# dspcraft/dsc

Hardware: AMD Instinct MI355X
Metric: batched 1-D rfft GSamples/s (higher is better)
Workload: dtype f32

## Files before the change

### dsc_amd/csrc/fft_c2c_32k.hip

```cpp
#define DSC_R2C64K_HELPERS_ONLY 1
#include "fft_r2c_64k.hip"

namespace {

template<bool INV, bool CAST>
__global__ __launch_bounds__(1024) void c2c32k_kernel(const f2 *__restrict__ z, f2 *__restrict__ Z, int batch, const f2 *__restrict__ aux,
                                                      int in_pitch, int in_len) {
    constexpr int EB = CAST ? 4 : 8;
    auto sample = [](__amdgpu_buffer_rsrc_t r, int voff, int soff) {
        if constexpr (CAST) return cf{__builtin_bit_cast(float, __builtin_amdgcn_raw_buffer_load_b32(r, voff, soff, kStream)), 0.0f};
        else return load_c(r, voff, soff);
    };
    extern __shared__ __attribute__((aligned(16))) float lds[];
    float *plane = lds;
    f2 *T = (f2 *) (lds + kPlaneFloats);
    fill_twiddle_table(T, aux);
    const int wave_sgpr = __builtin_amdgcn_readfirstlane(threadIdx.x >> 6);
    constexpr float kScale = 1.0f / (float) kM;

    cf v[32];
    {
        const int row0 = blockIdx.x;
        const __amdgpu_buffer_rsrc_t r0 = __builtin_amdgcn_make_buffer_rsrc(
            (void *) ((const char *) z + (size_t) row0 * in_pitch * EB), 0, row0 < batch ? in_len * EB : 0, 0x00020000);
        const int load_off = thread_id(wave_sgpr) * EB;
#pragma unroll
        for (int a = 0; a < 32; ++a) v[a] = sample(r0, load_off, a * 1024 * EB);
    }
    for (int row = blockIdx.x; row < batch; row += gridDim.x) {
        const int next_row = row + gridDim.x;
        const __amdgpu_buffer_rsrc_t rnext = __builtin_amdgcn_make_buffer_rsrc(
            (void *) ((const char *) z + (size_t) next_row * in_pitch * EB), 0, next_row < batch ? in_len * EB : 0, 0x00020000);
        const __amdgpu_buffer_rsrc_t rout = __builtin_amdgcn_make_buffer_rsrc((void *) (Z + (size_t) row * kM), 0, kM * 8, 0x00020000);
        three_passes<INV>(v, plane, T, aux, wave_sgpr, wave_sgpr, false, false);
        if (INV) {
#pragma unroll
            for (int p = 0; p < 32; ++p) v[p] = cf{v[p].x * kScale, v[p].y * kScale};
        }
        const int load_off = thread_id(wave_sgpr) * EB;
        staged_time_store(v, plane, rout, wave_sgpr, [&](bool first_half) {
            if (first_half) {
#pragma unroll
                for (int a = 0; a < 16; ++a) v[2 * a] = sample(rnext, load_off, a * 1024 * EB);
            } else {
#pragma unroll
                for (int a = 16; a < 32; ++a) v[2 * (a - 16) + 1] = sample(rnext, load_off, a * 1024 * EB);
            }
        });
        unzip_rows(v);
    }
}

}

void dsc_launch_fft32k_c32(const void *z, void *Z, int batch, int in_pitch, int in_len, bool inverse, bool cast, const void *aux, int n_cu,
                           hipStream_t stream) {
    if (batch <= 0) return;
    static unsigned long long attr_devices = 0;
    if (dsc_first_use_on_device(attr_devices)) {
        DSC_KERNEL_CHECK(hipFuncSetAttribute((const void *) c2c32k_kernel<false, false>, hipFuncAttributeMaxDynamicSharedMemorySize, kLdsBytes));
        DSC_KERNEL_CHECK(hipFuncSetAttribute((const void *) c2c32k_kernel<true, false>, hipFuncAttributeMaxDynamicSharedMemorySize, kLdsBytes));
        DSC_KERNEL_CHECK(hipFuncSetAttribute((const void *) c2c32k_kernel<false, true>, hipFuncAttributeMaxDynamicSharedMemorySize, kLdsBytes));
        DSC_KERNEL_CHECK(hipFuncSetAttribute((const void *) c2c32k_kernel<true, true>, hipFuncAttributeMaxDynamicSharedMemorySize, kLdsBytes));
    }
    const int grid = batch < n_cu ? batch : n_cu;
#define C2C32K(INV, CAST) DSC_LAUNCH((c2c32k_kernel<INV, CAST>), dim3(grid), dim3(1024), kLdsBytes, stream, (const f2 *) z, (f2 *) Z, batch, (const f2 *) aux, in_pitch, in_len)
    if (inverse) { if (cast) C2C32K(true, true); else C2C32K(true, false); }
    else         { if (cast) C2C32K(false, true); else C2C32K(false, false); }
#undef C2C32K
}
```

### dsc_amd/csrc/fft_r2c_64k.hip

```cpp
#include "kernels.h"

#include <hip/hip_runtime.h>

#include <cmath>
#include <cstdlib>
#include <utility>

namespace {

typedef float f2 __attribute__((ext_vector_type(2)));

struct cf { float x, y; };
__device__ __forceinline__ cf operator+(cf a, cf b) { return cf{a.x + b.x, a.y + b.y}; }
__device__ __forceinline__ cf operator-(cf a, cf b) { return cf{a.x - b.x, a.y - b.y}; }
__device__ __forceinline__ cf to_cf(f2 a) { return cf{a.x, a.y}; }
__device__ __forceinline__ f2 to_f2(cf a) { return f2{a.x, a.y}; }

constexpr int kM = 32768;
constexpr int kPlaneFloats = 1024 * 34;
constexpr int kLdsBytes = kPlaneFloats * 4 + 1024 * 8;
constexpr int kTabEntries = 1024;

constexpr int kAuxW1024 = 0, kAuxW32768 = 1024, kAuxW65536 = 2048, kAuxEntries = 3072;

// ... 144 lines not shown
__device__ __forceinline__ void dit_stage(cf (&v)[32], std::integer_sequence<int, G...>) {
    (dit_group<INV, S, G>(v, std::make_integer_sequence<int, (32 >> S)>{}), ...);
}

template<bool INV>
__device__ __forceinline__ void dft32(cf (&v)[32]) {
    dit_stage<INV, 1>(v, std::make_integer_sequence<int, 1>{});
    dit_stage<INV, 2>(v, std::make_integer_sequence<int, 2>{});
    dit_stage<INV, 3>(v, std::make_integer_sequence<int, 4>{});
    dit_stage<INV, 4>(v, std::make_integer_sequence<int, 8>{});
    dit_stage<INV, 5>(v, std::make_integer_sequence<int, 16>{});
}

template<bool INV>
__device__ __forceinline__ void dft32_head(cf (&v)[32]) {
    dit_stage<INV, 1>(v, std::make_integer_sequence<int, 1>{});
    dit_stage<INV, 2>(v, std::make_integer_sequence<int, 2>{});
}
template<bool INV, int Q>
__device__ __forceinline__ void dft32_quarter(cf (&v)[32]) {
    dit_stage<INV, 3>(v, std::integer_sequence<int, Q>{});
    dit_stage<INV, 4>(v, std::integer_sequence<int, 2 * Q, 2 * Q + 1>{});
    dit_stage<INV, 5>(v, std::integer_sequence<int, 4 * Q, 4 * Q + 1, 4 * Q + 2, 4 * Q + 3>{});
}
#endif

typedef unsigned int u2 __attribute__((ext_vector_type(2)));
typedef unsigned int u4 __attribute__((ext_vector_type(4)));
typedef float f4 __attribute__((ext_vector_type(4)));

#ifndef DSC_LDS_SPLIT_READS
#define DSC_LDS_SPLIT_READS 1
#endif
__device__ __forceinline__ f2 lds_read_b64(const f2 *p) {
#if DSC_LDS_SPLIT_READS
    return *(const volatile __attribute__((address_space(3))) f2 *) p;
#else
    return *p;
#endif
}

__device__ __forceinline__ void lds_barrier() {
    __builtin_amdgcn_fence(__ATOMIC_RELEASE, "workgroup", "local");
    __builtin_amdgcn_s_barrier();
    __builtin_amdgcn_fence(__ATOMIC_ACQUIRE, "workgroup", "local");
}

__device__ __forceinline__ float bperm(int byte_addr, float x) {
    return __int_as_float(__builtin_amdgcn_ds_bpermute(byte_addr, __float_as_int(x)));
}

__device__ __forceinline__ int column_of(int wave, int lane) {
    int kp = lane < 32 ? 32 * wave + lane : 1024 - 32 * wave - (63 - lane);
    return kp == 1024 ? 512 : kp;
}

#ifdef DSC_R2C64K_PROBE
#define PROBE_ARGS , int io_on
#define PROBE_NULL , 1
#define IO_ON io_on
#else
#define PROBE_ARGS
#define PROBE_NULL
#define IO_ON 1
#endif

__device__ __forceinline__ int thread_id(int wave_sgpr) {
    int zero;
    asm volatile("v_mov_b32 %0, 0" : "=v"(zero));
    const int lane = __builtin_amdgcn_mbcnt_hi(-1, __builtin_amdgcn_mbcnt_lo(-1, zero));
    return (wave_sgpr << 6) | lane;
}

#ifndef DSC_STREAM_AUX
#define DSC_STREAM_AUX 2
#endif
constexpr int kStream = DSC_STREAM_AUX;
__device__ __forceinline__ cf load_c(__amdgpu_buffer_rsrc_t r, int voff, int soff) {
    return to_cf(__builtin_bit_cast(f2, __builtin_amdgcn_raw_buffer_load_b64(r, voff, soff, kStream)));
}
#ifndef DSC_FILTER_EARLY_LOADS
#define DSC_FILTER_EARLY_LOADS 4
#endif
#ifndef DSC_IRFFT_PIN_PASS3
#define DSC_IRFFT_PIN_PASS3 1
#endif
#ifndef DSC_IRFFT_EARLY_PAIRS
#define DSC_IRFFT_EARLY_PAIRS 4
#endif
#ifndef DSC_IRFFT_LOAD_AUX
#define DSC_IRFFT_LOAD_AUX 0
#endif
__device__ __forceinline__ cf load_c_spec(__amdgpu_buffer_rsrc_t r, int voff, int soff) {
    return to_cf(__builtin_bit_cast(f2, __builtin_amdgcn_raw_buffer_load_b64(r, voff, soff, DSC_IRFFT_LOAD_AUX)));
}
__device__ __forceinline__ cf load_c_cached(__amdgpu_buffer_rsrc_t r, int voff, int soff) {
    return to_cf(__builtin_bit_cast(f2, __builtin_amdgcn_raw_buffer_load_b64(r, voff, soff, 0)));
}
template<int POLICY>
__device__ __forceinline__ void store_c(cf a, __amdgpu_buffer_rsrc_t r, int voff, int soff) {
    __builtin_amdgcn_raw_buffer_store_b64(__builtin_bit_cast(u2, to_f2(a)), r, voff, soff, POLICY);
}

__device__ __forceinline__ void fill_twiddle_table(f2 *T, const f2 *aux) {
    const int t = threadIdx.x;
    T[t] = aux[kAuxW1024 + (t >> 5) * (t & 31)];
    __syncthreads();
}

constexpr int kCPitch = 33;
static_assert(512 * kCPitch * 8 <= kPlaneFloats * 4, "the step buffer lives inside the plane");

__host__ __device__ constexpr int class_of(int k) { return (k ^ (k >> 1)) & 1; }
__host__ __device__ constexpr int index_in_class(int k) { return ((k >> 2) << 1) | (k & 1); }
static_assert(class_of(br5(0)) == 0 && class_of(br5(7)) == 0 && class_of(br5(24)) == 0 && class_of(br5(31)) == 0 &&
              class_of(br5(8)) == 1 && class_of(br5(23)) == 1, "class 0 = quarters 0 and 3 of a dft32 output");

__device__ __forceinline__ int reader_column(int t) {
    const int a = t >> 5;
    return (t & 31) | ((((a >> 3) | ((a & 7) << 2))) << 5);
}
__device__ __forceinline__ int spectrum_wave(int wave_sgpr) { return (wave_sgpr >> 2) | ((wave_sgpr & 3) << 2); }

template<int Q>
__device__ __forceinline__ void quarter_write(f2 *buf, int wbase, const cf (&v)[32]) {
    int wbase_hi = wbase + 8 * (32 * kCPitch);
    asm("" : "+v"(wbase_hi));
    f2 *lo8 = buf + wbase;
    f2 *hi8 = buf + wbase_hi;
#pragma unroll
    for (int p = 8 * Q; p < 8 * Q + 8; ++p)
        if (index_in_class(br5(p)) < 8) lo8[index_in_class(br5(p)) * (32 * kCPitch)] = to_f2(v[p]);
#pragma unroll
    for (int p = 8 * Q; p < 8 * Q + 8; ++p)
        if (index_in_class(br5(p)) >= 8) hi8[(index_in_class(br5(p)) - 8) * (32 * kCPitch)] = to_f2(v[p]);
}

__device__ __forceinline__ void step_read(const f2 *buf, int row, cf (&dst)[32]) {
    const f2 *r = buf + __mul24(row, kCPitch);
#pragma unroll
    for (int m = 0; m < 32; ++m) dst[m] = to_cf(lds_read_b64(r + m));
}

__device__ __forceinline__ void pin(cf (&v)[32]) {
#pragma unroll
    for (int p = 0; p < 32; p += 8)
        asm volatile("" : "+v"(v[p].x), "+v"(v[p].y), "+v"(v[p + 1].x), "+v"(v[p + 1].y), "+v"(v[p + 2].x), "+v"(v[p + 2].y), "+v"(v[p + 3].x),
                     "+v"(v[p + 3].y), "+v"(v[p + 4].x), "+v"(v[p + 4].y), "+v"(v[p + 5].x), "+v"(v[p + 5].y), "+v"(v[p + 6].x), "+v"(v[p + 6].y),
                     "+v"(v[p + 7].x), "+v"(v[p + 7].y));
}

template<typename Finish>
__device__ __forceinline__ void exchange(f2 *buf, int wbase, int rclass, int rrow, cf (&src)[32], cf (&dst)[32], Finish finish) {
    pin(src);
    lds_barrier();
    finish(std::integral_constant<int, 0>{});
    quarter_write<0>(buf, wbase, src);
    finish(std::integral_constant<int, 3>{});
    quarter_write<3>(buf, wbase, src);
    lds_barrier();
    cf r[32];
    if (rclass == 0) step_read(buf, rrow, r);
    finish(std::integral_constant<int, 1>{});
    lds_barrier();
    quarter_write<1>(buf, wbase, src);
    finish(std::integral_constant<int, 2>{});
    quarter_write<2>(buf, wbase, src);
    lds_barrier();
    if (rclass != 0) step_read(buf, rrow, r);
#pragma unroll
    for (int m = 0; m < 32; ++m) dst[m] = r[m];
}

struct no_hook { __device__ __forceinline__ void operator()() const {} };

template<bool INV, typename Hook = no_hook>
__device__ __forceinline__ void three_passes(cf (&v)[32], float *plane, const f2 *T, const f2 *aux, int wave_sgpr, int col_wave,
                                             bool mirrored_in, bool mirrored_out, Hook before_pass3 = Hook{}) {
    f2 *buf = (f2 *) plane;
    const int wave_class = ((wave_sgpr >> 2) ^ (wave_sgpr >> 3)) & 1;
    dft32_head<INV>(v);
    cf u[32];
    {
        const int t = thread_id(wave_sgpr);
        const int col = mirrored_in ? column_of(col_wave, t & 63) : t;
        const int hi = col >> 5;
        const f2 *th = T + hi;
        const int rc = reader_column(t);
        exchange(buf, __mul24(col & 31, kCPitch) + hi, wave_class, (index_in_class(rc >> 5) << 5) | (rc & 31), v, u, [&](auto Q) {
            constexpr int kQ = decltype(Q)::value;
            dft32_quarter<INV, kQ>(v);
#pragma unroll
            for (int p = 8 * kQ; p < 8 * kQ + 8; ++p) {
                if (p == 0) continue;
                const cf w = to_cf(th[32 * br5(p)]);
                v[p] = INV ? cmul_conj(v[p], w) : cmul(v[p], w);
            }
        });
    }
    dft32_head<INV>(u);
    {
        const int t = thread_id(wave_sgpr);
        const int rc = reader_column(t);
        const int hi = rc >> 5, lo = rc & 31;
        const cf tw2_base = to_cf(aux[kAuxW32768 + __mul24(hi, lo)]);
        const f2 *tl = T + lo;
        const int col_out = mirrored_out ? column_of(col_wave, t & 63) : rc;
        const int k2 = col_out >> 5;
        const int rclass = mirrored_out ? class_of(k2) : wave_class;
        exchange(buf, __mul24(hi, kCPitch) + lo, rclass, (index_in_class(k2) << 5) | (col_out & 31), u, v, [&](auto Q) {
            constexpr int kQ = decltype(Q)::value;
            dft32_quarter<INV, kQ>(u);
#ifdef DSC_DFT32_DIF
            constexpr bool kSumsOnly = false;
#else
            constexpr bool kSumsOnly = true;
#endif
#pragma unroll
            for (int p = 8 * kQ; p < 8 * kQ + 8; ++p) {
                const cf w = p == 0 ? tw2_base : cmul(tw2_base, to_cf(tl[32 * br5(p)]));
                if (kSumsOnly && p < 4) u[p] = twiddle_mul_second_fused<INV>(u[p], w);
                else u[p] = INV ? cmul_conj(u[p], w) : cmul(u[p], w);
            }
        });
    }
    before_pass3();
    dft32<INV>(v);
}

__device__ __forceinline__ void real_pair(cf p, cf q, cf wq, float hs, cf &out_k, cf &out_mk) {
    const cf s = cf{p.x + q.x, p.y - q.y};
    const cf d = cf{p.x - q.x, p.y + q.y};
    const cf wd = cmul(d, wq);
    out_k = cf{hs * s.x + wd.x, hs * s.y + wd.y};
    out_mk = cf{hs * s.x - wd.x, wd.y - hs * s.y};
}

__device__ __forceinline__ int partner_byte_addr(int wave, int lane) {
    return ((wave == 0 && (lane == 63 || lane == 0)) ? lane : 63 - lane) * 4;
}

#ifndef DSC_R2C64K_HELPERS_ONLY
__global__ __launch_bounds__(1024) void rfft64k_kernel(const float *__restrict__ x, f2 *__restrict__ X, int batch,
                                                       const f2 *__restrict__ aux, int in_pitch, int in_len PROBE_ARGS) {
    extern __shared__ __attribute__((aligned(16))) float lds[];
    float *plane = lds;
    f2 *T = (f2 *) (lds + kPlaneFloats);
    fill_twiddle_table(T, aux);

    const int wave_sgpr = __builtin_amdgcn_readfirstlane(threadIdx.x >> 6);

    cf v[32];
    {
        const int row0 = blockIdx.x;
        const __amdgpu_buffer_rsrc_t r0 = __builtin_amdgcn_make_buffer_rsrc(
            (void *) (x + (size_t) row0 * in_pitch), 0, row0 < batch ? in_len * 4 * IO_ON : 0, 0x00020000);
        const int load_off = thread_id(wave_sgpr) * 8;
#pragma unroll
        for (int j1 = 0; j1 < 32; ++j1) v[j1] = load_c(r0, load_off, j1 * 8192);
    }

    for (int row = blockIdx.x; row < batch; row += gridDim.x) {
        const int next_row = row + gridDim.x;
        const __amdgpu_buffer_rsrc_t rnext = __builtin_amdgcn_make_buffer_rsrc(
            (void *) (x + (size_t) next_row * in_pitch), 0, next_row < batch ? in_len * 4 * IO_ON : 0, 0x00020000);
        const __amdgpu_buffer_rsrc_t rout =
            __builtin_amdgcn_make_buffer_rsrc((void *) (X + (size_t) row * (kM + 1)), 0, (kM + 1) * 8 * IO_ON, 0x00020000);

        const int cw = spectrum_wave(wave_sgpr);
        three_passes<false>(v, plane, T, aux, wave_sgpr, cw, false, true);

        const int t4 = thread_id(wave_sgpr);
        const int lane = t4 & 63, wave = t4 >> 6;
        const int kp = column_of(cw, lane);
        const int partner_addr = partner_byte_addr(cw, lane);
        cf xk[16], xm[16];
        const cf zmid = v[br5(16)];
        if (cw == 0) {
#pragma unroll
            for (int r = 16; r < 31; ++r) v[br5(r)] = lane == 0 ? v[br5(r + 1)] : v[br5(r)];
            v[br5(31)] = lane == 0 ? v[br5(0)] : v[br5(31)];
        }
#pragma unroll
        for (int k3 = 0; k3 < 16; ++k3) {
            const int src = 31 - br5(k3);
            xm[k3].x = bperm(partner_addr, v[src].x);
            xm[k3].y = bperm(partner_addr, v[src].y);
        }
        {
            const cf wpost = to_cf(aux[kAuxW65536 + kp]);
            const cf post_base = cf{0.5f * wpost.y, -0.5f * wpost.x};
#pragma unroll
            for (int k3 = 0; k3 < 16; ++k3) {
                const cf c = cf{root64_re(k3), root64_im(k3)};
                const cf w = k3 == 0 ? post_base : cmul(post_base, c);
                real_pair(v[br5(k3)], xm[k3], w, 0.5f, xk[k3], xm[k3]);
            }
        }

        f2 *stage = (f2 *) plane;
        const int skew = (int) ((((size_t) (X + (size_t) row * (kM + 1))) >> 3) & 15);
        lds_barrier();
#pragma unroll
        for (int k3 = 0; k3 < 16; ++k3) stage[kp + 1024 * k3] = to_f2(xk[k3]);
        const cf xk15 = xk[15];
        const int load_off = thread_id(wave_sgpr) * 8;
#pragma unroll
        for (int j1 = 0; j1 < 16; ++j1) v[j1] = load_c(rnext, load_off, j1 * 8192);
        lds_barrier();
#pragma unroll
        for (int m = 0; m < 8; ++m) {
            const int k = 2 * (t4 + 1024 * m) - skew;
            if (m > 0 || k >= 0) {
                const f2 lo2 = lds_read_b64(stage + k), hi2 = lds_read_b64(stage + k + 1);
                const f4 q = f4{lo2.x, lo2.y, hi2.x, hi2.y};
                __builtin_amdgcn_raw_buffer_store_b128(__builtin_bit_cast(u4, q), rout, k * 8, 0, kStream);
            } else if (m == 0 && k == -1) {
                __builtin_amdgcn_raw_buffer_store_b64(__builtin_bit_cast(u2, stage[0]), rout, 0, 0, kStream);
            }
            if (m & 1) __builtin_amdgcn_sched_barrier(0);
        }
        lds_barrier();
        constexpr int kStage2 = kM / 2 - 16;
#pragma unroll
        for (int k3 = 0; k3 < 16; ++k3) stage[(kM - kStage2) - kp - 1024 * k3] = to_f2(xm[k3]);
        if (kp >= 1009) stage[kp + 15 * 1024 - kStage2] = to_f2(xk15);
        if (t4 == 0) stage[kM / 2 - kStage2] = f2{zmid.x, -zmid.y};
#pragma unroll
        for (int j1 = 16; j1 < 32; ++j1) v[j1] = load_c(rnext, load_off, j1 * 8192);
        lds_barrier();
#pragma unroll
        for (int m = 0; m < 9; ++m) {
            if (m == 8 && wave != 0) break;
            const int k = kM / 2 + 2 * (t4 + 1024 * m) - skew;
            if (m < 8 || k + 1 <= kM) {
                const f2 lo2 = lds_read_b64(stage + k - kStage2), hi2 = lds_read_b64(stage + k + 1 - kStage2);
                const f4 q = f4{lo2.x, lo2.y, hi2.x, hi2.y};
                __builtin_amdgcn_raw_buffer_store_b128(__builtin_bit_cast(u4, q), rout, k * 8, 0, kStream);
            } else if (m == 8 && k == kM) {
                __builtin_amdgcn_raw_buffer_store_b64(__builtin_bit_cast(u2, stage[k - kStage2]), rout, k * 8, 0, kStream);
            }
            if (m & 1) __builtin_amdgcn_sched_barrier(0);
        }
    }
}

#endif

__device__ __forceinline__ void inverse_prepass_direct(cf (&v)[32], cf y_mid, const f2 *aux, int wave_sgpr) {
    constexpr float kScale = 1.0f / (float) kM;
    const int t1 = thread_id(wave_sgpr);
    const int lane = t1 & 63, wave = t1 >> 6;
    const int c = column_of(wave, lane);
    const int partner_addr = partner_byte_addr(wave, lane);
    if (wave == 0 && lane == 0) { v[0].y = 0.f; v[16].y = 0.f; }
    const cf wpre = to_cf(aux[kAuxW65536 + c]);
    const cf wq_base = cf{0.5f * kScale * wpre.y, 0.5f * kScale * wpre.x};
#pragma unroll
    for (int half = 0; half < 2; ++half) {
        cf zm[8];
#pragma unroll
        for (int i = 0; i < 8; ++i) {
            const int a = half * 8 + i;
            const cf cj = cf{root64_re(a), -root64_im(a)};
            const cf wq = a == 0 ? wq_base : cmul(wq_base, cj);
            real_pair(v[a], v[16 + a], wq, 0.5f * kScale, v[a], zm[i]);
        }
#pragma unroll
        for (int i = 0; i < 8; ++i) {
            const int a = half * 8 + i;
            v[16 + a].x = bperm(partner_addr, zm[i].x);
            v[16 + a].y = bperm(partner_addr, zm[i].y);
        }
    }
    cf w[32];
#pragma unroll
    for (int r = 0; r < 16; ++r) { w[r] = v[r]; w[16 + r] = v[31 - r]; }
    if (wave == 0) {
#pragma unroll
        for (int r = 31; r > 16; --r) w[r] = lane == 0 ? w[r - 1] : w[r];
        w[16] = lane == 0 ? cf{kScale * y_mid.x, -kScale * y_mid.y} : w[16];
    }
#pragma unroll
    for (int r = 0; r < 32; ++r) v[r] = w[r];
}

template<typename IssueNext>
__device__ __forceinline__ void staged_time_store(cf (&v)[32], float *plane, __amdgpu_buffer_rsrc_t rout, int wave_sgpr,
                                                  IssueNext issue_next) {
    f2 *stage = (f2 *) plane;
    const int t4 = thread_id(wave_sgpr);
    const int c4 = reader_column(t4);
    lds_barrier();
#pragma unroll
    for (int p = 0; p < 32; p += 2) stage[c4 + 1024 * br5(p)] = to_f2(v[p]);
    issue_next(true);
    lds_barrier();
#pragma unroll
    for (int m = 0; m < 8; ++m) {
        const int k = 2 * (t4 + 1024 * m);
        const f2 lo2 = lds_read_b64(stage + k), hi2 = lds_read_b64(stage + k + 1);
        const f4 q = f4{lo2.x, lo2.y, hi2.x, hi2.y};
        __builtin_amdgcn_raw_buffer_store_b128(__builtin_bit_cast(u4, q), rout, k * 8, 0, kStream);
        if (m & 1) __builtin_amdgcn_sched_barrier(0);
    }
    lds_barrier();
#pragma unroll
    for (int p = 1; p < 32; p += 2) stage[c4 + 1024 * (br5(p) - 16)] = to_f2(v[p]);
    issue_next(false);
    lds_barrier();
#pragma unroll
    for (int m = 0; m < 8; ++m) {
        const int k = 2 * (t4 + 1024 * m);
        const f2 lo2 = lds_read_b64(stage + k), hi2 = lds_read_b64(stage + k + 1);
        const f4 q = f4{lo2.x, lo2.y, hi2.x, hi2.y};
        __builtin_amdgcn_raw_buffer_store_b128(__builtin_bit_cast(u4, q), rout, (kM / 2 + k) * 8, 0, kStream);
        if (m & 1) __builtin_amdgcn_sched_barrier(0);
    }
}

__device__ __forceinline__ void unzip_rows(cf (&v)[32]) {
    cf nxt[32];
#pragma unroll
    for (int a = 0; a < 16; ++a) { nxt[a] = v[2 * a]; nxt[16 + a] = v[2 * a + 1]; }
#pragma unroll
    for (int a = 0; a < 32; ++a) v[a] = nxt[a];
}

#ifndef DSC_R2C64K_HELPERS_ONLY
__global__ __launch_bounds__(1024) void irfft64k_kernel(const f2 *__restrict__ X, float *__restrict__ x, int batch,
                                                        const f2 *__restrict__ aux, int in_pitch, int in_len PROBE_ARGS) {
    extern __shared__ __attribute__((aligned(16))) float lds[];
    float *plane = lds;
    f2 *T = (f2 *) (lds + kPlaneFloats);
    fill_twiddle_table(T, aux);

    const int wave_sgpr = __builtin_amdgcn_readfirstlane(threadIdx.x >> 6);

    cf v[32];
    cf y_mid = cf{0.f, 0.f};
    {
        const int row0 = blockIdx.x;
        const __amdgpu_buffer_rsrc_t r0 = __builtin_amdgcn_make_buffer_rsrc(
            (void *) (X + (size_t) row0 * in_pitch), 0, row0 < batch ? in_len * 8 * IO_ON : 0, 0x00020000);
        const int t0 = thread_id(wave_sgpr);
        const int c = column_of(t0 >> 6, t0 & 63);
        const int pv = (kM - c - 15 * 1024) * 8;
#pragma unroll
        for (int a = 0; a < 16; ++a) {
            v[a] = load_c_spec(r0, c * 8, a * 8192);
            v[16 + a] = load_c_spec(r0, pv, (15 - a) * 8192);
        }
        if (c == 0) y_mid = load_c_spec(r0, (kM / 2) * 8, 0);
    }

    for (int row = blockIdx.x; row < batch; row += gridDim.x) {
        const int next_row = row + gridDim.x;
        const __amdgpu_buffer_rsrc_t rnext = __builtin_amdgcn_make_buffer_rsrc(
            (void *) (X + (size_t) next_row * in_pitch), 0, next_row < batch ? in_len * 8 * IO_ON : 0, 0x00020000);
        const __amdgpu_buffer_rsrc_t rout =
            __builtin_amdgcn_make_buffer_rsrc((void *) (x + (size_t) row * 65536), 0, 65536 * 4 * IO_ON, 0x00020000);

        inverse_prepass_direct(v, y_mid, aux, wave_sgpr);
        constexpr int kEarly = DSC_IRFFT_EARLY_PAIRS;
        cf early[kEarly > 0 ? 2 * kEarly : 1];
        three_passes<true>(v, plane, T, aux, wave_sgpr, wave_sgpr, true, false, [&]() {
            if constexpr (kEarly > 0) {
                const int t3 = thread_id(wave_sgpr);
                const int c3 = column_of(t3 >> 6, t3 & 63);
                const int pv3 = (kM - c3 - 15 * 1024) * 8;
#pragma unroll
                for (int a = 0; a < kEarly; ++a) {
                    early[2 * a] = load_c_spec(rnext, c3 * 8, a * 8192);
                    early[2 * a + 1] = load_c_spec(rnext, pv3, (15 - a) * 8192);
                }
            }
        });

#if DSC_IRFFT_PIN_PASS3
#pragma unroll
        for (int p = 0; p < 32; p += 8)
            asm volatile("" : "+v"(v[p].x), "+v"(v[p].y), "+v"(v[p + 1].x), "+v"(v[p + 1].y), "+v"(v[p + 2].x), "+v"(v[p + 2].y), "+v"(v[p + 3].x),
                         "+v"(v[p + 3].y), "+v"(v[p + 4].x), "+v"(v[p + 4].y), "+v"(v[p + 5].x), "+v"(v[p + 5].y), "+v"(v[p + 6].x), "+v"(v[p + 6].y),
                         "+v"(v[p + 7].x), "+v"(v[p + 7].y));
#endif
        const int t4 = thread_id(wave_sgpr);
        const int c = column_of(t4 >> 6, t4 & 63);
        const int pv = (kM - c - 15 * 1024) * 8;
        staged_time_store(v, plane, rout, wave_sgpr, [&](bool first_half) {
            if (first_half) {
                y_mid = cf{0.f, 0.f};
                if (c == 0) y_mid = load_c_spec(rnext, (kM / 2) * 8, 0);
#pragma unroll
                for (int i = 0; i < 8; ++i) {
                    v[2 * i] = load_c_spec(rnext, c * 8, (kEarly + i) * 8192);
                    v[16 + 2 * i] = load_c_spec(rnext, pv, (15 - kEarly - i) * 8192);
                }
            } else {
#pragma unroll
                for (int i = 0; i < 8 - kEarly; ++i) {
                    v[2 * i + 1] = load_c_spec(rnext, c * 8, (kEarly + 8 + i) * 8192);
                    v[17 + 2 * i] = load_c_spec(rnext, pv, (7 - kEarly - i) * 8192);
                }
            }
        });
        {
            cf nxt[32];
#pragma unroll
            for (int a = 0; a < 16; ++a) {
                if (a < kEarly)          { nxt[a] = early[2 * a];             nxt[16 + a] = early[2 * a + 1]; }
                else if (a < kEarly + 8) { nxt[a] = v[2 * (a - kEarly)];      nxt[16 + a] = v[16 + 2 * (a - kEarly)]; }
                else                     { nxt[a] = v[2 * (a - kEarly - 8) + 1]; nxt[16 + a] = v[17 + 2 * (a - kEarly - 8)]; }
            }
#pragma unroll
            for (int a = 0; a < 32; ++a) v[a] = nxt[a];
        }
    }
}

__global__ __launch_bounds__(1024) void filter64k_kernel(const float *__restrict__ x, const f2 *__restrict__ H,
                                                         float *__restrict__ y, int batch, const f2 *__restrict__ aux, int in_pitch,
                                                         int in_len) {
    extern __shared__ __attribute__((aligned(16))) float lds[];
    float *plane = lds;
    f2 *T = (f2 *) (lds + kPlaneFloats);
    fill_twiddle_table(T, aux);

    const int wave_sgpr = __builtin_amdgcn_readfirstlane(threadIdx.x >> 6);
    const __amdgpu_buffer_rsrc_t rh = __builtin_amdgcn_make_buffer_rsrc((void *) H, 0, (kM + 1) * 8, 0x00020000);
    constexpr float kScale = 1.0f / (float) kM;

    cf v[32];
    {
        const int row0 = blockIdx.x;
        const __amdgpu_buffer_rsrc_t r0 = __builtin_amdgcn_make_buffer_rsrc(
            (void *) (x + (size_t) row0 * in_pitch), 0, row0 < batch ? in_len * 4 : 0, 0x00020000);
        const int load_off = thread_id(wave_sgpr) * 8;
#pragma unroll
        for (int j1 = 0; j1 < 32; ++j1) v[j1] = load_c(r0, load_off, j1 * 8192);
    }
    for (int row = blockIdx.x; row < batch; row += gridDim.x) {
        const int next_row = row + gridDim.x;
        const __amdgpu_buffer_rsrc_t rnext = __builtin_amdgcn_make_buffer_rsrc(
            (void *) (x + (size_t) next_row * in_pitch), 0, next_row < batch ? in_len * 4 : 0, 0x00020000);
        const __amdgpu_buffer_rsrc_t rout =
            __builtin_amdgcn_make_buffer_rsrc((void *) (y + (size_t) row * 65536), 0, 65536 * 4, 0x00020000);
        const int cw = spectrum_wave(wave_sgpr);
        three_passes<false>(v, plane, T, aux, wave_sgpr, cw, false, true);

        {
            const int t1 = thread_id(wave_sgpr);
            const int lane = t1 & 63, wave = cw;
            const int c = column_of(wave, lane);
            const int partner_addr = partner_byte_addr(wave, lane);
            const cf wc = to_cf(aux[kAuxW65536 + c]);
            const cf post_base = cf{0.5f * wc.y, -0.5f * wc.x};
            const cf pre_base = cf{0.5f * kScale * wc.y, 0.5f * kScale * wc.x};
            if (wave == 0) {
                const cf zmid = v[br5(16)];
                const cf hmid = load_c_cached(rh, (kM / 2) * 8, 0);
                const cf pmid = cmul(cf{zmid.x, -zmid.y}, hmid);
                v[br5(16)] = lane == 0 ? cf{kScale * pmid.x, -kScale * pmid.y} : v[br5(16)];
            }
            cf park = v[br5(16)];
            if (wave == 0) {
#pragma unroll
                for (int r = 16; r < 31; ++r) v[br5(r)] = lane == 0 ? v[br5(r + 1)] : v[br5(r)];
                v[br5(31)] = lane == 0 ? v[br5(0)] : v[br5(31)];
            }
#pragma unroll
            for (int part = 0; part < 8; ++part) {
                cf q[2], zm[2];
#pragma unroll
                for (int i = 0; i < 2; ++i) {
                    const int a = part * 2 + i;
                    q[i].x = bperm(partner_addr, v[br5(31 - a)].x);
                    q[i].y = bperm(partner_addr, v[br5(31 - a)].y);
                }
#pragma unroll
                for (int i = 0; i < 2; ++i) {
                    const int a = part * 2 + i;
                    const cf w64 = cf{root64_re(a), root64_im(a)};
                    cf xk, xm;
                    real_pair(v[br5(a)], q[i], a == 0 ? post_base : cmul(post_base, w64), 0.5f, xk, xm);
                    const cf hk = load_c_cached(rh, c * 8, a * 8192);
                    const cf hm = load_c_cached(rh, (kM - 15 * 1024 - c) * 8, (15 - a) * 8192);
                    cf pk = cmul(xk, hk), pm = cmul(xm, hm);
                    if (a == 0) {
                        pk.y = (c == 0) ? 0.f : pk.y;
                        pm.y = (c == 0) ? 0.f : pm.y;
                    }
                    const cf w64c = cf{root64_re(a), -root64_im(a)};
                    real_pair(pk, pm, a == 0 ? pre_base : cmul(pre_base, w64c), 0.5f * kScale, v[br5(a)], zm[i]);
                }
#pragma unroll
                for (int i = 0; i < 2; ++i) {
                    const int a = part * 2 + i;
                    v[br5(31 - a)].x = bperm(partner_addr, zm[i].x);
                    v[br5(31 - a)].y = bperm(partner_addr, zm[i].y);
                }
                __builtin_amdgcn_sched_barrier(0);
            }
            if (wave == 0) {
#pragma unroll
                for (int r = 31; r > 16; --r) v[br5(r)] = lane == 0 ? v[br5(r - 1)] : v[br5(r)];
                v[br5(16)] = lane == 0 ? park : v[br5(16)];
            }
        }
        cf z[32];
#pragma unroll
        for (int r = 0; r < 32; ++r) z[r] = v[br5(r)];
        constexpr int kEarlyX = DSC_FILTER_EARLY_LOADS;
        cf early[kEarlyX > 0 ? kEarlyX : 1];
        three_passes<true>(z, plane, T, aux, wave_sgpr, cw, true, false, [&]() {
            if constexpr (kEarlyX > 0) {
                const int off = thread_id(wave_sgpr) * 8;
#pragma unroll
                for (int j1 = 0; j1 < kEarlyX; ++j1) early[j1] = load_c(rnext, off, j1 * 8192);
            }
        });
        {
            const int load_off = thread_id(wave_sgpr) * 8;
            staged_time_store(z, plane, rout, wave_sgpr, [&](bool first_half) {
                if (first_half) {
#pragma unroll
                    for (int i = 0; i < 16; ++i) z[2 * i] = load_c(rnext, load_off, (kEarlyX + i) * 8192);
                } else {
#pragma unroll
                    for (int i = 0; i < 16 - kEarlyX; ++i) z[2 * i + 1] = load_c(rnext, load_off, (kEarlyX + 16 + i) * 8192);
                }
            });
#pragma unroll
            for (int j1 = 0; j1 < 32; ++j1) v[j1] = j1 < kEarlyX ? early[j1] : j1 < kEarlyX + 16 ? z[2 * (j1 - kEarlyX)] : z[2 * (j1 - kEarlyX - 16) + 1];
        }
    }
}

#endif

}

#ifndef DSC_R2C64K_HELPERS_ONLY
size_t dsc_r2c64k_table_bytes() { return (size_t) kAuxEntries * sizeof(float) * 2; }

void dsc_r2c64k_build_tables(void *host_dst) {
    float *o = (float *) host_dst;
    auto put = [&](int at, long long k, long long n) {
        const long double a = -2.0L * 3.14159265358979323846264338327950288L * (long double) k / (long double) n;
        o[2 * at] = (float) cosl(a);
        o[2 * at + 1] = (float) sinl(a);
    };
    for (int m = 0; m < kTabEntries; ++m) {
        put(kAuxW1024 + m, m, 1024);
        put(kAuxW32768 + m, m, 32768);
        put(kAuxW65536 + m, m, 65536);
    }
    o[2 * (kAuxW1024 + 256)] = 0.f;  o[2 * (kAuxW1024 + 256) + 1] = -1.f;
    o[2 * (kAuxW1024 + 512)] = -1.f; o[2 * (kAuxW1024 + 512) + 1] = 0.f;
    o[2 * (kAuxW1024 + 768)] = 0.f;  o[2 * (kAuxW1024 + 768) + 1] = 1.f;
}

void dsc_launch_rfft64k(const float *x, void *X, int batch, int in_pitch, int in_len, const void *aux, int n_cu, hipStream_t stream) {
    if (batch <= 0) return;
    static unsigned long long attr_devices = 0;
    if (dsc_first_use_on_device(attr_devices)) {
        DSC_KERNEL_CHECK(hipFuncSetAttribute((const void *) rfft64k_kernel, hipFuncAttributeMaxDynamicSharedMemorySize, kLdsBytes));
    }
    const int grid = batch < n_cu ? batch : n_cu;
    DSC_LAUNCH(rfft64k_kernel, dim3(grid), dim3(1024), kLdsBytes, stream, x, (f2 *) X, batch, (const f2 *) aux, in_pitch, in_len PROBE_NULL);
}

void dsc_launch_irfft64k(const void *X, float *x, int batch, int in_pitch, int in_len, const void *aux, int n_cu, hipStream_t stream) {
    if (batch <= 0) return;
    static unsigned long long attr_devices = 0;
    if (dsc_first_use_on_device(attr_devices)) {
        DSC_KERNEL_CHECK(hipFuncSetAttribute((const void *) irfft64k_kernel, hipFuncAttributeMaxDynamicSharedMemorySize, kLdsBytes));
    }
    const int grid = batch < n_cu ? batch : n_cu;
    DSC_LAUNCH(irfft64k_kernel, dim3(grid), dim3(1024), kLdsBytes, stream, (const f2 *) X, x, batch, (const f2 *) aux, in_pitch, in_len PROBE_NULL);
}
void dsc_launch_filter64k(const float *s, const void *H, float *y, int batch, int in_pitch, int in_len, const void *aux, int n_cu,
                          hipStream_t stream) {
    if (batch <= 0) return;
    static unsigned long long attr_devices = 0;
    if (dsc_first_use_on_device(attr_devices)) {
        DSC_KERNEL_CHECK(hipFuncSetAttribute((const void *) filter64k_kernel, hipFuncAttributeMaxDynamicSharedMemorySize, kLdsBytes));
    }
    const int grid = batch < n_cu ? batch : n_cu;
    DSC_LAUNCH(filter64k_kernel, dim3(grid), dim3(1024), kLdsBytes, stream, s, (const f2 *) H, y, batch, (const f2 *) aux, in_pitch, in_len);
}
#endif
```

Before: 674.4.

## Split final DFT32 pass by output class and overlap with staged stores in rfft

The rfft64k kernel no longer runs the last dft32 pass as a whole. It computes the head, then the quarters in class order, and post-processes and stages one class of spectrum bins at a time. The second class's quarter DFTs and post-pair work are interleaved with the global stores of the first class, and next-row loads are split at a tunable early-load count. The aim is to hide the tail compute and LDS staging behind memory stores. In exchange it adds more complex index bookkeeping for skewed output alignment and a boundary-run fixup, plus possible register pressure from the extra nxt buffer. Similar by-class store paths are added behind flags, default off, for c2c, irfft and filter.

```diff
diff --git a/dsc_amd/csrc/fft_c2c_32k.hip b/dsc_amd/csrc/fft_c2c_32k.hip
--- a/dsc_amd/csrc/fft_c2c_32k.hip
+++ b/dsc_amd/csrc/fft_c2c_32k.hip
@@ -32,22 +32,27 @@
         const __amdgpu_buffer_rsrc_t rnext = __builtin_amdgcn_make_buffer_rsrc(
             (void *) ((const char *) z + (size_t) next_row * in_pitch * EB), 0, next_row < batch ? in_len * EB : 0, 0x00020000);
         const __amdgpu_buffer_rsrc_t rout = __builtin_amdgcn_make_buffer_rsrc((void *) (Z + (size_t) row * kM), 0, kM * 8, 0x00020000);
-        three_passes<INV>(v, plane, T, aux, wave_sgpr, wave_sgpr, false, false);
-        if (INV) {
+        three_passes<INV, !DSC_C2C_STORE_BY_CLASS>(v, plane, T, aux, wave_sgpr, wave_sgpr, false, false);
+        auto scale = [&](cf (&w)[32], int first, int last) {
+            if (INV) {
 #pragma unroll
-            for (int p = 0; p < 32; ++p) v[p] = cf{v[p].x * kScale, v[p].y * kScale};
-        }
+                for (int p = first; p < last; ++p) w[p] = cf{w[p].x * kScale, w[p].y * kScale};
+            }
+        };
         const int load_off = thread_id(wave_sgpr) * EB;
-        staged_time_store(v, plane, rout, wave_sgpr, [&](bool first_half) {
-            if (first_half) {
+        cf nxt[32];
+        auto issue_next = [&](bool first_half) {
 #pragma unroll
-                for (int a = 0; a < 16; ++a) v[2 * a] = sample(rnext, load_off, a * 1024 * EB);
-            } else {
+            for (int a = first_half ? 0 : 16; a < (first_half ? 16 : 32); ++a) nxt[a] = sample(rnext, load_off, a * 1024 * EB);
+        };
+#if DSC_C2C_STORE_BY_CLASS
+        staged_time_store_by_class<INV>(v, plane, rout, wave_sgpr, scale, issue_next);
+#else
+        scale(v, 0, 32);
+        staged_time_store(v, plane, rout, wave_sgpr, issue_next);
+#endif
 #pragma unroll
-                for (int a = 16; a < 32; ++a) v[2 * (a - 16) + 1] = sample(rnext, load_off, a * 1024 * EB);
-            }
-        });
-        unzip_rows(v);
+        for (int a = 0; a < 32; ++a) v[a] = nxt[a];
     }
 }
 
diff --git a/dsc_amd/csrc/fft_r2c_64k.hip b/dsc_amd/csrc/fft_r2c_64k.hip
--- a/dsc_amd/csrc/fft_r2c_64k.hip
+++ b/dsc_amd/csrc/fft_r2c_64k.hip
@@ -250,6 +250,18 @@
 #ifndef DSC_FILTER_EARLY_LOADS
 #define DSC_FILTER_EARLY_LOADS 4
 #endif
+#ifndef DSC_RFFT_EARLY_LOADS
+#define DSC_RFFT_EARLY_LOADS 12
+#endif
+#ifndef DSC_IRFFT_STORE_BY_CLASS
+#define DSC_IRFFT_STORE_BY_CLASS 0
+#endif
+#ifndef DSC_FILTER_STORE_BY_CLASS
+#define DSC_FILTER_STORE_BY_CLASS 0
+#endif
+#ifndef DSC_C2C_STORE_BY_CLASS
+#define DSC_C2C_STORE_BY_CLASS 0
+#endif
 #ifndef DSC_IRFFT_PIN_PASS3
 #define DSC_IRFFT_PIN_PASS3 1
 #endif
@@ -281,6 +293,7 @@
 
 __host__ __device__ constexpr int class_of(int k) { return (k ^ (k >> 1)) & 1; }
 __host__ __device__ constexpr int index_in_class(int k) { return ((k >> 2) << 1) | (k & 1); }
+__host__ __device__ constexpr int staged_row(int r) { return ((r >> 2) << 1) | ((r >> 1) & 1); }
 static_assert(class_of(br5(0)) == 0 && class_of(br5(7)) == 0 && class_of(br5(24)) == 0 && class_of(br5(31)) == 0 &&
               class_of(br5(8)) == 1 && class_of(br5(23)) == 1, "class 0 = quarters 0 and 3 of a dft32 output");
 
@@ -342,7 +355,7 @@
 
 struct no_hook { __device__ __forceinline__ void operator()() const {} };
 
-template<bool INV, typename Hook = no_hook>
+template<bool INV, bool PASS3 = true, typename Hook = no_hook>
 __device__ __forceinline__ void three_passes(cf (&v)[32], float *plane, const f2 *T, const f2 *aux, int wave_sgpr, int col_wave,
                                              bool mirrored_in, bool mirrored_out, Hook before_pass3 = Hook{}) {
     f2 *buf = (f2 *) plane;
@@ -393,7 +406,7 @@
         });
     }
     before_pass3();
-    dft32<INV>(v);
+    if constexpr (PASS3) dft32<INV>(v);
 }
 
 __device__ __forceinline__ void real_pair(cf p, cf q, cf wq, float hs, cf &out_k, cf &out_mk) {
@@ -409,6 +422,93 @@
 }
 
 #ifndef DSC_R2C64K_HELPERS_ONLY
+__host__ __device__ constexpr int pair_of(int cls, int i) { return 4 * (i >> 1) + (cls == 0 ? 3 * (i & 1) : 1 + (i & 1)); }
+__host__ __device__ constexpr int pair_of_column0(int cls, int i) { return 4 * (i >> 1) + (i & 1) + 2 * cls; }
+static_assert(class_of(pair_of(0, 1)) == 0 && class_of(31 - pair_of(0, 1)) == 0 && class_of(pair_of(1, 6)) == 1 &&
+              class_of(32 - pair_of_column0(0, 1)) == 0 && class_of(32 - pair_of_column0(1, 7)) == 1 &&
+              staged_row(3) == 1 && staged_row(2) == 1 && staged_row(31) == 15 && staged_row(32) == 16, "classes of the output rows");
+
+template<int CLS>
+__device__ __forceinline__ void post_pairs_fetch(const cf (&v)[32], int partner_addr, cf (&xm)[8]) {
+#pragma unroll
+    for (int i = 0; i < 8; ++i) {
+        const int src = 31 - br5(pair_of(CLS, i));
+        xm[i].x = bperm(partner_addr, v[src].x);
+        xm[i].y = bperm(partner_addr, v[src].y);
+    }
+}
+template<int CLS>
+__device__ __forceinline__ void post_pairs_finish(const cf (&v)[32], cf post_base, cf (&xk)[8], cf (&xm)[8]) {
+    asm volatile("" : "+v"(post_base.x), "+v"(post_base.y));
+#pragma unroll
+    for (int i = 0; i < 8; ++i) {
+        const int k3 = pair_of(CLS, i);
+        const cf c = cf{root64_re(k3), root64_im(k3)};
+        const cf w = k3 == 0 ? post_base : cmul(post_base, c);
+        real_pair(v[br5(k3)], xm[i], w, 0.5f, xk[i], xm[i]);
+    }
+}
+
+template<int CLS, bool COLUMN0>
+__device__ __forceinline__ void stage_class(f2 *stage, int kp, int lane, const cf (&xk)[8], const cf (&xm)[8]) {
+#pragma unroll
+    for (int i = 0; i < 8; ++i) stage[kp + 1024 * staged_row(pair_of(CLS, i))] = to_f2(xk[i]);
+#pragma unroll
+    for (int i = 0; i < 8; ++i) {
+        int at = (1024 - kp) + 1024 * staged_row(31 - pair_of(CLS, i));
+        if (COLUMN0) at = lane == 0 ? 1024 * staged_row(32 - pair_of_column0(CLS, i)) : at;
+        stage[at] = to_f2(xm[i]);
+    }
+}
+
+template<int CLS, typename Slice>
+__device__ __forceinline__ void store_class(const f2 *stage, __amdgpu_buffer_rsrc_t rout, int t, int skew, Slice slice) {
+    constexpr int kDropped = 1 << 30;
+    const int odd = t >> 9;
+    const int kl = 2 * (t & 511) - skew;
+    const int first = (CLS == 0 ? 3 * odd : 1 + odd) * 1024 + kl;
+    const int at = odd * 1024 + kl;
+    const bool joined = odd == CLS;
+    const int off = (kl >= 0 || joined) ? first * 8 : kDropped;
+#pragma unroll
+    for (int g = 0; g < 4; ++g) {
+        f2 lo2[2], hi2[2];
+#pragma unroll
+        for (int h = 0; h < 2; ++h) {
+            const int m = 2 * g + h;
+            const f2 *src = stage + (CLS == 0 && m == 0 ? max(at, 0) : at) + 2048 * m;
+            lo2[h] = lds_read_b64(src);
+            hi2[h] = lds_read_b64(src + 1);
+        }
+        __builtin_amdgcn_sched_barrier(0);
+        slice(g);
+        __builtin_amdgcn_sched_barrier(0);
+#pragma unroll
+        for (int h = 0; h < 2; ++h) {
+            const int m = 2 * g + h;
+            const f4 q = f4{lo2[h].x, lo2[h].y, hi2[h].x, hi2[h].y};
+            const u4 data = __builtin_bit_cast(u4, q);
+            __builtin_amdgcn_raw_buffer_store_b128(data, rout, CLS == 0 && m == 0 ? (kl >= 0 ? first * 8 : kDropped) : off, m * 32768, kStream);
+            asm volatile("s_nop 1" : : "v"(data));
+        }
+        __builtin_amdgcn_sched_barrier(0);
+    }
+    constexpr int kRuns = CLS == 0 ? 9 : 8;
+    const int jt = t >> 4, i = t & 15, jh = t - 192;
+    const bool last = CLS == 0 && jt == 8;
+    const bool is_tail = jt < kRuns && i < skew + (last ? 1 : 0);
+    const bool is_head = jh >= 0 && jh < kRuns && (skew & 1);
+    if (is_tail || is_head) {
+        const int end_staged = CLS == 0 ? (last ? 16 * 1024 : (2 * jt + 1) * 1024) : (2 * jt + 2) * 1024;
+        const int end_bin = CLS == 0 ? (last ? kM : 4096 * jt + 1024) : 4096 * jt + 3072;
+        const int start_staged = CLS == 0 ? (jh == 0 ? 0 : (2 * jh - 1) * 1024) : 2 * jh * 1024;
+        const int start_bin = CLS == 0 ? (jh == 0 ? 0 : 4096 * jh - 1024) : 4096 * jh + 1024;
+        const int from = is_head ? start_staged : end_staged - skew + i;
+        const int bin = is_head ? start_bin : end_bin - skew + i;
+        __builtin_amdgcn_raw_buffer_store_b64(__builtin_bit_cast(u2, stage[from]), rout, bin * 8, 0, kStream);
+    }
+}
+
 __global__ __launch_bounds__(1024) void rfft64k_kernel(const float *__restrict__ x, f2 *__restrict__ X, int batch,
                                                        const f2 *__restrict__ aux, int in_pitch, int in_len PROBE_ARGS) {
     extern __shared__ __attribute__((aligned(16))) float lds[];
@@ -436,80 +536,97 @@
             __builtin_amdgcn_make_buffer_rsrc((void *) (X + (size_t) row * (kM + 1)), 0, (kM + 1) * 8 * IO_ON, 0x00020000);
 
         const int cw = spectrum_wave(wave_sgpr);
-        three_passes<false>(v, plane, T, aux, wave_sgpr, cw, false, true);
-
+        three_passes<false, false>(v, plane, T, aux, wave_sgpr, cw, false, true);
+
+        dft32_head<false>(v);
+        pin(v);
         const int t4 = thread_id(wave_sgpr);
-        const int lane = t4 & 63, wave = t4 >> 6;
+        const int lane = t4 & 63;
         const int kp = column_of(cw, lane);
         const int partner_addr = partner_byte_addr(cw, lane);
-        cf xk[16], xm[16];
-        const cf zmid = v[br5(16)];
+        const cf wpost = to_cf(aux[kAuxW65536 + kp]);
+        const cf post_base = cf{0.5f * wpost.y, -0.5f * wpost.x};
+        cf ak[8], am[8];
+        cf zmid = cf{0.f, 0.f};
         if (cw == 0) {
+            dft32_quarter<false, 0>(v);
+            dft32_quarter<false, 3>(v);
+            dft32_quarter<false, 1>(v);
+            dft32_quarter<false, 2>(v);
+            zmid = v[br5(16)];
 #pragma unroll
             for (int r = 16; r < 31; ++r) v[br5(r)] = lane == 0 ? v[br5(r + 1)] : v[br5(r)];
             v[br5(31)] = lane == 0 ? v[br5(0)] : v[br5(31)];
-        }
-#pragma unroll
-        for (int k3 = 0; k3 < 16; ++k3) {
-            const int src = 31 - br5(k3);
-            xm[k3].x = bperm(partner_addr, v[src].x);
-            xm[k3].y = bperm(partner_addr, v[src].y);
-        }
-        {
-            const cf wpost = to_cf(aux[kAuxW65536 + kp]);
-            const cf post_base = cf{0.5f * wpost.y, -0.5f * wpost.x};
-#pragma unroll
-            for (int k3 = 0; k3 < 16; ++k3) {
-                const cf c = cf{root64_re(k3), root64_im(k3)};
-                const cf w = k3 == 0 ? post_base : cmul(post_base, c);
-                real_pair(v[br5(k3)], xm[k3], w, 0.5f, xk[k3], xm[k3]);
+            cf bk[8], bm[8];
+            __builtin_amdgcn_sched_barrier(0);
+            post_pairs_fetch<0>(v, partner_addr, am);
+            post_pairs_finish<0>(v, post_base, ak, am);
+            __builtin_amdgcn_sched_barrier(0);
+            post_pairs_fetch<1>(v, partner_addr, bm);
+            post_pairs_finish<1>(v, post_base, bk, bm);
+            __builtin_amdgcn_sched_barrier(0);
+            cf zm[16];
+#pragma unroll
+            for (int i = 0; i < 8; ++i) { zm[pair_of(0, i)] = am[i]; zm[pair_of(1, i)] = bm[i]; }
+#pragma unroll
+            for (int i = 0; i < 8; ++i) {
+                am[i] = lane == 0 ? zm[pair_of_column0(0, i)] : am[i];
+                bm[i] = lane == 0 ? zm[pair_of_column0(1, i)] : bm[i];
             }
+#pragma unroll
+            for (int i = 0; i < 8; ++i) { v[8 + i] = bk[i]; v[16 + i] = bm[i]; }
+        } else {
+            dft32_quarter<false, 0>(v);
+            dft32_quarter<false, 3>(v);
+            post_pairs_fetch<0>(v, partner_addr, am);
+            post_pairs_finish<0>(v, post_base, ak, am);
         }
 
         f2 *stage = (f2 *) plane;
         const int skew = (int) ((((size_t) (X + (size_t) row * (kM + 1))) >> 3) & 15);
+        constexpr int kEarlyLoads = DSC_RFFT_EARLY_LOADS;
+        cf nxt[32];
         lds_barrier();
-#pragma unroll
-        for (int k3 = 0; k3 < 16; ++k3) stage[kp + 1024 * k3] = to_f2(xk[k3]);
-        const cf xk15 = xk[15];
-        const int load_off = thread_id(wave_sgpr) * 8;
-#pragma unroll
-        for (int j1 = 0; j1 < 16; ++j1) v[j1] = load_c(rnext, load_off, j1 * 8192);
+        if (cw == 0) {
+            stage_class<0, true>(stage, kp, lane, ak, am);
+            if (lane == 0) stage[1024 * staged_row(16)] = f2{zmid.x, -zmid.y};
+        } else {
+            stage_class<0, false>(stage, kp, lane, ak, am);
+        }
+        {
+            const int load_off = thread_id(wave_sgpr) * 8;
+#pragma unroll
+            for (int j1 = 0; j1 < kEarlyLoads; ++j1) nxt[j1] = load_c(rnext, load_off, j1 * 8192);
+        }
         lds_barrier();
-#pragma unroll
-        for (int m = 0; m < 8; ++m) {
-            const int k = 2 * (t4 + 1024 * m) - skew;
-            if (m > 0 || k >= 0) {
-                const f2 lo2 = lds_read_b64(stage + k), hi2 = lds_read_b64(stage + k + 1);
-                const f4 q = f4{lo2.x, lo2.y, hi2.x, hi2.y};
-                __builtin_amdgcn_raw_buffer_store_b128(__builtin_bit_cast(u4, q), rout, k * 8, 0, kStream);
-            } else if (m == 0 && k == -1) {
-                __builtin_amdgcn_raw_buffer_store_b64(__builtin_bit_cast(u2, stage[0]), rout, 0, 0, kStream);
+        store_class<0>(stage, rout, thread_id(wave_sgpr), skew, [&](int g) {
+            if (cw != 0) {
+                if (g == 0) dft32_quarter<false, 1>(v);
+                if (g == 1) dft32_quarter<false, 2>(v);
+                if (g == 2) {
+                    cf ck[8], cm[8];
+                    post_pairs_fetch<1>(v, partner_addr, cm);
+                    post_pairs_finish<1>(v, post_base, ck, cm);
+#pragma unroll
+                    for (int i = 0; i < 8; ++i) { v[8 + i] = ck[i]; v[16 + i] = cm[i]; }
+                }
             }
-            if (m & 1) __builtin_amdgcn_sched_barrier(0);
-        }
+        });
+        cf bk[8], bm[8];
+#pragma unroll
+        for (int i = 0; i < 8; ++i) { bk[i] = v[8 + i]; bm[i] = v[16 + i]; }
         lds_barrier();
-        constexpr int kStage2 = kM / 2 - 16;
-#pragma unroll
-        for (int k3 = 0; k3 < 16; ++k3) stage[(kM - kStage2) - kp - 1024 * k3] = to_f2(xm[k3]);
-        if (kp >= 1009) stage[kp + 15 * 1024 - kStage2] = to_f2(xk15);
-        if (t4 == 0) stage[kM / 2 - kStage2] = f2{zmid.x, -zmid.y};
-#pragma unroll
-        for (int j1 = 16; j1 < 32; ++j1) v[j1] = load_c(rnext, load_off, j1 * 8192);
+        if (cw == 0) stage_class<1, true>(stage, kp, lane, bk, bm);
+        else stage_class<1, false>(stage, kp, lane, bk, bm);
+        {
+            const int load_off = thread_id(wave_sgpr) * 8;
+#pragma unroll
+            for (int j1 = kEarlyLoads; j1 < 32; ++j1) nxt[j1] = load_c(rnext, load_off, j1 * 8192);
+        }
         lds_barrier();
-#pragma unroll
-        for (int m = 0; m < 9; ++m) {
-            if (m == 8 && wave != 0) break;
-            const int k = kM / 2 + 2 * (t4 + 1024 * m) - skew;
-            if (m < 8 || k + 1 <= kM) {
-                const f2 lo2 = lds_read_b64(stage + k - kStage2), hi2 = lds_read_b64(stage + k + 1 - kStage2);
-                const f4 q = f4{lo2.x, lo2.y, hi2.x, hi2.y};
-                __builtin_amdgcn_raw_buffer_store_b128(__builtin_bit_cast(u4, q), rout, k * 8, 0, kStream);
-            } else if (m == 8 && k == kM) {
-                __builtin_amdgcn_raw_buffer_store_b64(__builtin_bit_cast(u2, stage[k - kStage2]), rout, k * 8, 0, kStream);
-            }
-            if (m & 1) __builtin_amdgcn_sched_barrier(0);
-        }
+        store_class<1>(stage, rout, thread_id(wave_sgpr), skew, [](int) {});
+#pragma unroll
+        for (int j1 = 0; j1 < 32; ++j1) v[j1] = nxt[j1];
     }
 }
 
@@ -587,6 +704,70 @@
     }
 }
 
+
+template<int CLS, typename Slice>
+__device__ __forceinline__ void time_store_class(const f2 *stage, __amdgpu_buffer_rsrc_t rout, int t, Slice slice) {
+    const int odd = t >> 9;
+    const f2 *src = stage + (odd * 1024 + 2 * (t & 511));
+    const int off = ((CLS == 0 ? 3 * odd : 1 + odd) * 1024 + 2 * (t & 511)) * 8;
+#pragma unroll
+    for (int g = 0; g < 4; ++g) {
+        f2 lo2[2], hi2[2];
+#pragma unroll
+        for (int h = 0; h < 2; ++h) {
+            lo2[h] = lds_read_b64(src + 2048 * (2 * g + h));
+            hi2[h] = lds_read_b64(src + 2048 * (2 * g + h) + 1);
+        }
+        __builtin_amdgcn_sched_barrier(0);
+        slice(g);
+        __builtin_amdgcn_sched_barrier(0);
+#pragma unroll
+        for (int h = 0; h < 2; ++h) {
+            const u4 data = __builtin_bit_cast(u4, f4{lo2[h].x, lo2[h].y, hi2[h].x, hi2[h].y});
+            __builtin_amdgcn_raw_buffer_store_b128(data, rout, off, (2 * g + h) * 32768, kStream);
+            asm volatile("s_nop 1" : : "v"(data));
+        }
+        __builtin_amdgcn_sched_barrier(0);
+    }
+}
+
+struct no_finish { __device__ __forceinline__ void operator()(cf (&)[32], int, int) const {} };
+
+template<bool INV, typename Finish, typename IssueNext>
+__device__ __forceinline__ void staged_time_store_by_class(cf (&v)[32], float *plane, __amdgpu_buffer_rsrc_t rout, int wave_sgpr,
+                                                           Finish finish, IssueNext issue_next) {
+    f2 *stage = (f2 *) plane;
+    dft32_head<INV>(v);
+    pin(v);
+    dft32_quarter<INV, 0>(v);
+    finish(v, 0, 8);
+    dft32_quarter<INV, 3>(v);
+    finish(v, 24, 32);
+    lds_barrier();
+    {
+        f2 *col = stage + reader_column(thread_id(wave_sgpr));
+#pragma unroll
+        for (int p = 0; p < 8; ++p) col[1024 * staged_row(br5(p))] = to_f2(v[p]);
+#pragma unroll
+        for (int p = 24; p < 32; ++p) col[1024 * staged_row(br5(p))] = to_f2(v[p]);
+    }
+    issue_next(true);
+    lds_barrier();
+    time_store_class<0>(stage, rout, thread_id(wave_sgpr), [&](int g) {
+        if (g == 0) { dft32_quarter<INV, 1>(v); finish(v, 8, 16); }
+        if (g == 1) { dft32_quarter<INV, 2>(v); finish(v, 16, 24); }
+    });
+    lds_barrier();
+    {
+        f2 *col = stage + reader_column(thread_id(wave_sgpr));
+#pragma unroll
+        for (int p = 8; p < 24; ++p) col[1024 * staged_row(br5(p))] = to_f2(v[p]);
+    }
+    issue_next(false);
+    lds_barrier();
+    time_store_class<1>(stage, rout, thread_id(wave_sgpr), [](int) {});
+}
+
 __device__ __forceinline__ void unzip_rows(cf (&v)[32]) {
     cf nxt[32];
 #pragma unroll
@@ -632,7 +813,7 @@
         inverse_prepass_direct(v, y_mid, aux, wave_sgpr);
         constexpr int kEarly = DSC_IRFFT_EARLY_PAIRS;
         cf early[kEarly > 0 ? 2 * kEarly : 1];
-        three_passes<true>(v, plane, T, aux, wave_sgpr, wave_sgpr, true, false, [&]() {
+        three_passes<true, !DSC_IRFFT_STORE_BY_CLASS>(v, plane, T, aux, wave_sgpr, wave_sgpr, true, false, [&]() {
             if constexpr (kEarly > 0) {
                 const int t3 = thread_id(wave_sgpr);
                 const int c3 = column_of(t3 >> 6, t3 & 63);
@@ -645,7 +826,7 @@
             }
         });
 
-#if DSC_IRFFT_PIN_PASS3
+#if DSC_IRFFT_PIN_PASS3 && !DSC_IRFFT_STORE_BY_CLASS
 #pragma unroll
         for (int p = 0; p < 32; p += 8)
             asm volatile("" : "+v"(v[p].x), "+v"(v[p].y), "+v"(v[p + 1].x), "+v"(v[p + 1].y), "+v"(v[p + 2].x), "+v"(v[p + 2].y), "+v"(v[p + 3].x),
@@ -655,33 +836,34 @@
         const int t4 = thread_id(wave_sgpr);
         const int c = column_of(t4 >> 6, t4 & 63);
         const int pv = (kM - c - 15 * 1024) * 8;
-        staged_time_store(v, plane, rout, wave_sgpr, [&](bool first_half) {
+        cf ld[32];
+        auto issue_next = [&](bool first_half) {
             if (first_half) {
                 y_mid = cf{0.f, 0.f};
                 if (c == 0) y_mid = load_c_spec(rnext, (kM / 2) * 8, 0);
 #pragma unroll
                 for (int i = 0; i < 8; ++i) {
-                    v[2 * i] = load_c_spec(rnext, c * 8, (kEarly + i) * 8192);
-                    v[16 + 2 * i] = load_c_spec(rnext, pv, (15 - kEarly - i) * 8192);
+                    ld[2 * i] = load_c_spec(rnext, c * 8, (kEarly + i) * 8192);
+                    ld[16 + 2 * i] = load_c_spec(rnext, pv, (15 - kEarly - i) * 8192);
                 }
             } else {
 #pragma unroll
                 for (int i = 0; i < 8 - kEarly; ++i) {
-                    v[2 * i + 1] = load_c_spec(rnext, c * 8, (kEarly + 8 + i) * 8192);
-                    v[17 + 2 * i] = load_c_spec(rnext, pv, (7 - kEarly - i) * 8192);
+                    ld[2 * i + 1] = load_c_spec(rnext, c * 8, (kEarly + 8 + i) * 8192);
+                    ld[17 + 2 * i] = load_c_spec(rnext, pv, (7 - kEarly - i) * 8192);
                 }
             }
-        });
-        {
-            cf nxt[32];
-#pragma unroll
-            for (int a = 0; a < 16; ++a) {
-                if (a < kEarly)          { nxt[a] = early[2 * a];             nxt[16 + a] = early[2 * a + 1]; }
-                else if (a < kEarly + 8) { nxt[a] = v[2 * (a - kEarly)];      nxt[16 + a] = v[16 + 2 * (a - kEarly)]; }
-                else                     { nxt[a] = v[2 * (a - kEarly - 8) + 1]; nxt[16 + a] = v[17 + 2 * (a - kEarly - 8)]; }
-            }
-#pragma unroll
-            for (int a = 0; a < 32; ++a) v[a] = nxt[a];
+        };
+#if DSC_IRFFT_STORE_BY_CLASS
+        staged_time_store_by_class<true>(v, plane, rout, wave_sgpr, no_finish{}, issue_next);
+#else
+        staged_time_store(v, plane, rout, wave_sgpr, issue_next);
+#endif
+#pragma unroll
+        for (int a = 0; a < 16; ++a) {
+            if (a < kEarly)          { v[a] = early[2 * a];              v[16 + a] = early[2 * a + 1]; }
+            else if (a < kEarly + 8) { v[a] = ld[2 * (a - kEarly)];      v[16 + a] = ld[16 + 2 * (a - kEarly)]; }
+            else                     { v[a] = ld[2 * (a - kEarly - 8) + 1]; v[16 + a] = ld[17 + 2 * (a - kEarly - 8)]; }
         }
     }
 }
@@ -780,7 +962,7 @@
         for (int r = 0; r < 32; ++r) z[r] = v[br5(r)];
         constexpr int kEarlyX = DSC_FILTER_EARLY_LOADS;
         cf early[kEarlyX > 0 ? kEarlyX : 1];
-        three_passes<true>(z, plane, T, aux, wave_sgpr, cw, true, false, [&]() {
+        three_passes<true, !DSC_FILTER_STORE_BY_CLASS>(z, plane, T, aux, wave_sgpr, cw, true, false, [&]() {
             if constexpr (kEarlyX > 0) {
                 const int off = thread_id(wave_sgpr) * 8;
 #pragma unroll
@@ -789,17 +971,22 @@
         });
         {
             const int load_off = thread_id(wave_sgpr) * 8;
-            staged_time_store(z, plane, rout, wave_sgpr, [&](bool first_half) {
+            auto issue_next = [&](bool first_half) {
                 if (first_half) {
 #pragma unroll
-                    for (int i = 0; i < 16; ++i) z[2 * i] = load_c(rnext, load_off, (kEarlyX + i) * 8192);
+                    for (int i = 0; i < 16; ++i) v[kEarlyX + i] = load_c(rnext, load_off, (kEarlyX + i) * 8192);
                 } else {
 #pragma unroll
-                    for (int i = 0; i < 16 - kEarlyX; ++i) z[2 * i + 1] = load_c(rnext, load_off, (kEarlyX + 16 + i) * 8192);
+                    for (int i = 0; i < 16 - kEarlyX; ++i) v[kEarlyX + 16 + i] = load_c(rnext, load_off, (kEarlyX + 16 + i) * 8192);
                 }
-            });
-#pragma unroll
-            for (int j1 = 0; j1 < 32; ++j1) v[j1] = j1 < kEarlyX ? early[j1] : j1 < kEarlyX + 16 ? z[2 * (j1 - kEarlyX)] : z[2 * (j1 - kEarlyX - 16) + 1];
+            };
+#if DSC_FILTER_STORE_BY_CLASS
+            staged_time_store_by_class<true>(z, plane, rout, wave_sgpr, no_finish{}, issue_next);
+#else
+            staged_time_store(z, plane, rout, wave_sgpr, issue_next);
+#endif
+#pragma unroll
+            for (int j1 = 0; j1 < kEarlyX; ++j1) v[j1] = early[j1];
         }
     }
 }
```

Result: slower. 665.7 (-1.3%).
